# BoMingZhao/GaussianPrediction

Measured on AMD Instinct MI355X. Metric: rendered views/s (full train step) @1M Gaussians 1352x1014, higher is better.
Workload: dtype f32; 1 GPU; configs[2]: HyperNeRF-like 1M Gaussians, 1352x1014, stage-3 full train step (deform, raster, L1+SSIM loss, Adam: all HIP kernels); gaussians=1000000, width=1352, height=1014, keypoints=250, nearest_num=6, parallelism=view-parallel x1, ranks_seen_by_rccl=1, self_launched=False

## Files before the change

### gaussianprediction_amd/csrc/deform_kernels.h

```cpp
#pragma once
#include "gp_common.h"
#include "loss_adam_kernels.h"

struct MlpDev {
    long rows;
    int in_dim, in_pad, out_dim;
    int feature_dim, xyz_freq, time_freq;
    const float* w[5];
    const float* b[5];
    const float* feature;
    const float* xyz;
    const float* t;
    const float* pk;
};

struct MlpPackLayout {
    int q0;
    int tb0;
    long off_f[4], off_b[4], total;
};
static inline __host__ __device__ MlpPackLayout mlp_pack_layout(int in_dim) {
    MlpPackLayout L;
    L.q0 = (in_dim + 15) / 16;
    L.tb0 = 2 * ((in_dim + 31) / 32);
// ... 69 lines not shown
__global__ __launch_bounds__(1024) void gp_blend_bwd_reduce_kernel(const float* __restrict__ partial, int nblocks, int KA,
                                                                  int od, float* __restrict__ g_delta);
__global__ __launch_bounds__(256) void gp_act_fwd_kernel(long n, const float* __restrict__ scaling_raw,
                                                         const float* __restrict__ opacity_raw,
                                                         const float* __restrict__ delta_o, int stride, float beta,
                                                         float* __restrict__ scale, float* __restrict__ opacity);
__global__ __launch_bounds__(256) void gp_act_bwd_kernel(long n, const float* __restrict__ scaling_raw,
                                                         const float* __restrict__ opacity_raw,
                                                         const float* __restrict__ delta_o, int stride, float beta,
                                                         const float* __restrict__ g_scale,
                                                         const float* __restrict__ g_opacity,
                                                         float* __restrict__ g_scaling_raw, float* __restrict__ g_opacity_raw,
                                                         float* __restrict__ g_delta_o);

__global__ __launch_bounds__(512) void gp_mlp_bwd_weight5_kernel(MlpWeightJobs t, long rows);
__global__ __launch_bounds__(512) void gp_mlp_fwd_small_kernel(MlpDev p, float* __restrict__ out, float* __restrict__ saved_x,
                                                               float* __restrict__ saved_h);
__global__ __launch_bounds__(512) void gp_mlp_bwd_data_small_kernel(MlpDev p, const float* __restrict__ saved_h,
                                                                    const float* __restrict__ dL_dout, float* __restrict__ dz,
                                                                    float* __restrict__ dfeature, float* __restrict__ dxyz);

__global__ __launch_bounds__(256) void gp_mlp_fwd_split_small_kernel(MlpDev p, float* __restrict__ out, float* __restrict__ saved_x, float* hx,
                                                                     uint32_t* flags, uint32_t* err);
__global__ __launch_bounds__(256) void gp_mlp_fwd_split_small_agent_kernel(MlpDev p, float* __restrict__ out, float* __restrict__ saved_x,
                                                                           float* hx, uint32_t* flags, uint32_t* err);
__global__ __launch_bounds__(256) void gp_mlp_bwd_data_split_small_kernel(MlpDev p, const float* __restrict__ saved_h, const float* __restrict__ dL_dout,
                                                                          float* dz, float* __restrict__ dfeature, float* __restrict__ dxyz, float* gx,
                                                                          uint32_t* flags, uint32_t* err, int form);
struct AdamTable;
__global__ __launch_bounds__(512) void gp_mlp_bwd_data_small_adam_kernel(MlpDev p, const float* __restrict__ saved_h,
// ... 15 lines not shown
```

### gaussianprediction_amd/csrc/deform_kernels.hip

```cpp
#include "gp_common.h"
#include "deform_kernels.h"

typedef float f32x16 __attribute__((ext_vector_type(16)));

#define MLP_ROWS 32
#define MLP_THREADS 512
#define MLP_W 256

__device__ __forceinline__ int act_idx(int f, int j) { return f * MLP_ROWS + (j ^ (f & 31)); }
__device__ __forceinline__ int cd_row(int r, int half) { return (r & 3) + 8 * (r >> 2) + 4 * half; }

__device__ __forceinline__ void build_input(float* buf, const MlpDev& p, long row0, int tid) {
    const int fd = p.feature_dim, xf = p.xyz_freq, tf = p.time_freq;
    for (int e = tid; e < fd * MLP_ROWS; e += MLP_THREADS) {
        const int jj = e / fd, f = e - jj * fd;
        const long row = row0 + jj;
        buf[act_idx(f, jj)] = row < p.rows ? p.feature[row * fd + f] : 0.f;
    }
    for (int e = tid; e < 3 * xf * MLP_ROWS; e += MLP_THREADS) {
        const int jj = e % MLP_ROWS, cf = e / MLP_ROWS;
        const int c = cf / xf, fr = cf - c * xf;
        const long row = row0 + jj;
        float sv = 0.f, cv = 0.f;
        if (row < p.rows) {
// ... 407 lines not shown
                        for (int fr = 0; fr < p.xyz_freq; ++fr) {
                            const float sc = (float)(1u << fr);
                            float sv, cv;
                            sincosf(x * sc, &sv, &cv);
                            const int f = p.feature_dim + 2 * (c * p.xyz_freq + fr);
                            g += sc * (cv * buf[act_idx(f, jj)] - sv * buf[act_idx(f + 1, jj)]);
                        }
                        dxyz[row * 3 + c] = g;
                    }
                }
            }
        }
    }
}

__device__ __forceinline__ void mlp_bwd_weight_body(const float* __restrict__ dZ, int n_out, const float* __restrict__ H, int ldh,
                                                    int n_in, long rows, long rows_per_block, float* __restrict__ dW, int lddw,
                                                    float* __restrict__ db, int row_block, int n_row_blocks, int bz, int by) {
    __shared__ float s_red[8][16][64];
    __shared__ float s_b[8][32];
    const int tid = threadIdx.x, lane = tid & 63, wave = tid >> 6, half = lane >> 5, j = lane & 31;
    const int o = 32 * bz + j;
    const int i = 32 * by + j;
    const long b_begin = (long)row_block * rows_per_block;
    long b_end = b_begin + rows_per_block;
    if (b_end > rows) b_end = rows;
    long per_wave = ((b_end - b_begin + 7) / 8 + 1) & ~1L;
    const long r_begin = b_begin + wave * per_wave;
    long r_end = r_begin + per_wave;
    if (r_end > b_end) r_end = b_end;
    f32x16 acc;
#pragma unroll
    for (int r = 0; r < 16; ++r) acc[r] = 0.f;
// ... 5 lines not shown
        for (int u = 0; u < 4; ++u) {
            const long r = rb + 2 * u + half;
            a[u] = (r < r_end && o_ok) ? dZ[r * n_out + o] : 0.f;
            b[u] = (r < r_end && i_ok) ? H[r * (long)ldh + i] : 0.f;
            bsum += a[u];
        }
#pragma unroll
        for (int u = 0; u < 4; ++u) acc = __builtin_amdgcn_mfma_f32_32x32x2f32(a[u], b[u], acc, 0, 0, 0);
    }
#pragma unroll
    for (int r = 0; r < 16; ++r) s_red[wave][r][lane] = acc[r];
    bsum += __shfl_xor(bsum, 32);
    if (half == 0) s_b[wave][j] = bsum;
    __syncthreads();
    const bool single = n_row_blocks == 1;
    for (int e = tid; e < 16 * 64; e += MLP_THREADS) {
        const int r = e >> 6, l = e & 63;
        float v = 0.f;
#pragma unroll
        for (int w = 0; w < 8; ++w) v += s_red[w][r][l];
        const int oo = 32 * bz + cd_row(r, l >> 5), ii = 32 * by + (l & 31);
        if (oo < n_out && ii < n_in) {
            float* dst = &dW[(size_t)oo * lddw + ii];
            if (single) *dst += v; else atomicAdd(dst, v);
        }
    }
    if (db && by == 0 && tid < 32) {
        float v = 0.f;
#pragma unroll
        for (int w = 0; w < 8; ++w) v += s_b[w][tid];
        const int oo = 32 * bz + tid;
        if (oo < n_out) { if (single) db[oo] += v; else atomicAdd(&db[oo], v); }
    }
}

__global__ __launch_bounds__(MLP_THREADS) void gp_mlp_bwd_weight_kernel(const float* __restrict__ dZ, int n_out,
                                                                        const float* __restrict__ H, int ldh, int n_in,
                                                                        long rows, long rows_per_block,
                                                                        float* __restrict__ dW, int lddw,
                                                                        float* __restrict__ db) {
    mlp_bwd_weight_body(dZ, n_out, H, ldh, n_in, rows, rows_per_block, dW, lddw, db, blockIdx.x, gridDim.x, blockIdx.z, blockIdx.y);
}
__global__ __launch_bounds__(MLP_THREADS) void gp_mlp_bwd_weight5_kernel(MlpWeightJobs t, long rows) {
    const int l = blockIdx.x;
    if ((int)blockIdx.y * 32 >= t.n_in[l] || (int)blockIdx.z * 32 >= t.n_out[l]) return;
    mlp_bwd_weight_body(t.dZ[l], t.n_out[l], t.H[l], t.ldh[l], t.n_in[l], rows, rows, t.dW[l], t.n_in[l], t.db[l], 0, 1, blockIdx.z,
                        blockIdx.y);
}

__global__ __launch_bounds__(256) void gp_mlp_bwd_weight64_kernel(const float* __restrict__ dZ, int n_out, const float* __restrict__ H,
                                                                 int ldh, int n_in, long rows, long rows_per_block,
                                                                 unsigned n_row_blocks, float* __restrict__ dW, int lddw,
                                                                 float* __restrict__ db) {
    __shared__ float s_red[4][4][16][64];
    const int tid = threadIdx.x, lane = tid & 63, wave = tid >> 6, half = lane >> 5, j = lane & 31;
    const int n_ib = (n_in + 63) / 64;
    const int ntp = n_ib * ((n_out + 63) / 64);
    const unsigned flat = blockIdx.x, xcd = flat & 7u, seq = flat >> 3;
    const unsigned slab = (seq / ntp) * 8u + xcd, tp = seq % ntp;
    if (slab >= n_row_blocks) return;
    const int o0 = 64 * (tp / n_ib), i0 = 64 * (tp % n_ib);
    const long b_begin = (long)slab * rows_per_block;
// ... 436 lines not shown
            extern __shared__ float s_dyn[];
            double* s_tot = (double*)(((uintptr_t)s_dyn + 7) & ~(uintptr_t)7);
            loss_finalize_body(r.fin, (float*)(s_tot + 8), s_tot);
        } else {
            adam_chunk_body<256>(r.t, blockIdx.x - r.fin_blocks, threadIdx.x, r.b1, r.b2, r.eps, r.zero_grad, r.skip_flag);
        }
        return;
    }
    blend_bwd_body<NN, I16>(a, g_xyz_t, g_q_t, g_delta, g_raw_w, g_xyz, g_rot, partial, blockIdx.x - riders, gridDim.x - riders);
}
__global__ __launch_bounds__(256) void gp_blend_bwd6_ride_kernel(BlendRideDev r, BB_ARGS) { blend_bwd_ride_body<6, false>(r, a, g_xyz_t, g_q_t, g_delta, g_raw_w, g_xyz, g_rot, partial); }
__global__ __launch_bounds__(256) void gp_blend_bwd8_ride_kernel(BlendRideDev r, BB_ARGS) { blend_bwd_ride_body<8, false>(r, a, g_xyz_t, g_q_t, g_delta, g_raw_w, g_xyz, g_rot, partial); }
__global__ __launch_bounds__(256) void gp_blend_bwd6_i16_ride_kernel(BlendRideDev r, BB_ARGS) { blend_bwd_ride_body<6, true>(r, a, g_xyz_t, g_q_t, g_delta, g_raw_w, g_xyz, g_rot, partial); }
__global__ __launch_bounds__(256) void gp_blend_bwd8_i16_ride_kernel(BlendRideDev r, BB_ARGS) { blend_bwd_ride_body<8, true>(r, a, g_xyz_t, g_q_t, g_delta, g_raw_w, g_xyz, g_rot, partial); }

__global__ __launch_bounds__(1024) void gp_blend_bwd_reduce_kernel(const float* __restrict__ partial, int nblocks, int KA,
                                                                  int od, float* __restrict__ g_delta) {
    __shared__ float s_r[16][64];
    const int lane = threadIdx.x & 63, wave = threadIdx.x >> 6;
    const int e = blockIdx.x * 64 + lane;
    float v0 = 0.f, v1 = 0.f, v2 = 0.f, v3 = 0.f;
    if (e < KA) {
        int b = wave;
        for (; b + 240 < nblocks; b += 256) {
            float t[16];
#pragma unroll
            for (int u = 0; u < 16; ++u) t[u] = partial[(size_t)(b + 16 * u) * KA + e];
#pragma unroll
            for (int u = 0; u < 16; u += 4) { v0 += t[u]; v1 += t[u + 1]; v2 += t[u + 2]; v3 += t[u + 3]; }
        }
        for (; b + 48 < nblocks; b += 64) {
            v0 += partial[(size_t)b * KA + e]; v1 += partial[(size_t)(b + 16) * KA + e];
            v2 += partial[(size_t)(b + 32) * KA + e]; v3 += partial[(size_t)(b + 48) * KA + e];
        }
        for (; b < nblocks; b += 16) v0 += partial[(size_t)b * KA + e];
    }
    s_r[wave][lane] = (v0 + v1) + (v2 + v3);
    __syncthreads();
    if (wave == 0 && e < KA) {
        float t = 0.f;
#pragma unroll
        for (int w = 0; w < 16; ++w) t += s_r[w][lane];
        g_delta[(size_t)(e / 7) * od + (e % 7)] = t;
        if (e % 7 == 6) for (int c = 7; c < od; ++c) g_delta[(size_t)(e / 7) * od + c] = 0.f;
    }
}

__device__ __forceinline__ float sigmoidf(float x) { return 1.f / (1.f + expf(-x)); }

__global__ __launch_bounds__(256) void gp_act_fwd_kernel(long n, const float* __restrict__ scaling_raw,
                                                        const float* __restrict__ opacity_raw,
                                                        const float* __restrict__ delta_o, int stride, float beta,
                                                        float* __restrict__ scale, float* __restrict__ opacity) {
    const long i = (long)blockIdx.x * 256 + threadIdx.x;
    if (i >= n) return;
    const float s0 = scaling_raw[3 * i], s1 = scaling_raw[3 * i + 1], s2 = scaling_raw[3 * i + 2];
    const float op_raw = opacity_raw[i];
    const float dlt = delta_o ? delta_o[i * stride] : 0.f;
    scale[3 * i] = expf(s0);
    scale[3 * i + 1] = expf(s1);
// ... 32 lines not shown
```

### gaussianprediction_amd/csrc/gp_capi_deform.hip

```cpp
#include "gp_common.h"
#include "deform_kernels.h"
#include "loss_adam_kernels.h"
#include <stdlib.h>

static int make_mlp(const gp_mlp_params* p, const gp_mlp_input* x, MlpDev& m) {
    if (!p || !x) GP_FAIL("null mlp params/input");
    if (p->width != 256 || p->depth != 4) GP_FAIL("Deformable_Field: only d=4, w=256 is implemented (got d=%d w=%d)", p->depth, p->width);
    if (p->out_dim < 7 || p->out_dim > 8) GP_FAIL("out_dim must be 7 or 8 (got %d)", p->out_dim);
    if (x->feature_dim <= 0 || x->feature_dim % 4 || x->xyz_freq < 0 || x->xyz_freq > 16 || x->time_freq < 0 || x->time_freq > 16)
        GP_FAIL("bad input encoding dims");
    const int in_dim = x->feature_dim + 6 * x->xyz_freq + 2 * x->time_freq;
    if (in_dim != p->in_dim) GP_FAIL("in_dim %d != feature_dim + 6*xyz_freq + 2*time_freq = %d", p->in_dim, in_dim);
    if (in_dim % 4 || in_dim > 256) GP_FAIL("in_dim %d must be a multiple of 4 and <= 256", in_dim);
    if (x->rows < 0) GP_FAIL("negative rows");
    for (int l = 0; l < 5; ++l)
        if (!p->w[l] || !p->b[l]) GP_FAIL("null weight pointer (layer %d)", l);
    if (x->rows > 0 && (!x->feature || (x->xyz_freq > 0 && !x->xyz) || (x->time_freq > 0 && !x->t))) GP_FAIL("null input pointer");
    m.rows = x->rows; m.in_dim = in_dim; m.in_pad = (in_dim + 7) / 8 * 8; m.out_dim = p->out_dim;
    m.feature_dim = x->feature_dim; m.xyz_freq = x->xyz_freq; m.time_freq = x->time_freq;
    for (int l = 0; l < 5; ++l) { m.w[l] = p->w[l]; m.b[l] = p->b[l]; }
    m.feature = x->feature; m.xyz = x->xyz; m.t = x->t;
    m.pk = p->packed;
    if (m.pk && ((uintptr_t)m.pk & 15) != 0) GP_FAIL("gp_mlp_params.packed must be 16-byte aligned");
    if (p->scratch && ((uintptr_t)p->scratch & 15) != 0) GP_FAIL("gp_mlp_params.scratch must be 16-byte aligned");
// ... 96 lines not shown
            hipLaunchKernelGGL(gp_mlp_fwd_kernel, dim3(gp_blocks((size_t)m.rows, 32)), dim3(512), 0, (hipStream_t)stream_, m, out, sx, sh);
    GP_LAUNCH_CHECK(); }
    return 0;
}

bool gp_mlp_backward_splits(const gp_mlp_params* p, int64_t rows) {
    if (!p) return false;
    MlpDev m;
    memset(&m, 0, sizeof(m));
    m.rows = rows;
    int mode = 0;
    int* st = nullptr;
    return mlp_split_grid(m, p->scratch, mode, st) != 0 && (mode == 1 || mode == 3);
}

int gp_mlp_backward_impl(const gp_mlp_params* p, const gp_mlp_input* x, const float* acts, const float* dL_dout, gp_mlp_grads* g,
                         float* dL_dfeature, float* dL_dxyz, gp_alloc_fn alloc, void* alloc_ctx, gp_stream_t stream_, GpAdamRider* rider,
                         bool accumulate_dfeature) {
    hipStream_t s = (hipStream_t)stream_;
    MlpDev m;
    if (make_mlp(p, x, m)) return 1;
    if (m.rows == 0) return 0;
    if (!acts || !dL_dout || !g || !alloc) GP_FAIL("null argument");
    for (int l = 0; l < 5; ++l)
        if (!g->dw[l] || !g->db[l]) GP_FAIL("null weight-grad pointer (layer %d)", l);
    const float* sx = acts;
    const float* sh = acts + gp_align_up(acts_x_floats(m), 64);
    const size_t dz_bytes = gp_align_up((size_t)4 * m.rows * 256 * sizeof(float), 256);
    float* dz = (float*)alloc(alloc_ctx, GP_BUF_TEMP, dz_bytes);
    if (!dz) GP_FAIL("allocator returned NULL for TEMP (%zu B)", dz_bytes);
    int split_mode = 0;
    int* split_state = nullptr;
    const unsigned split = mlp_split_grid(m, p->scratch, split_mode, split_state);
    if (split && (split_mode == 1 || split_mode == 3)) {
        float* gx = (float*)((char*)p->scratch + GP_MLP_SCRATCH_FLAG_BYTES);
        uint32_t* flags = (uint32_t*)p->scratch;
        GpProfScope _p("mlp_bwd_data", s);
        hipLaunchKernelGGL(gp_mlp_bwd_data_split_small_kernel, dim3(split), dim3(256), 0, s, m, sh, dL_dout, dz, dL_dfeature, dL_dxyz, gx, flags,
                           flags + GP_MLP_SCRATCH_ERR_WORD, (split_mode == 3 ? 1 : 0) | (accumulate_dfeature ? 2 : 0));
        GP_LAUNCH_CHECK();
    } else if (m.rows <= GP_MLP_SMALL_ROWS && rider && rider->armed) {
        rider->armed = false;
        const unsigned n_mlp = gp_blocks((size_t)m.rows, 16);
        GpProfScope _p("adam", s);
        hipLaunchKernelGGL(gp_mlp_bwd_data_small_adam_kernel, dim3(n_mlp + rider->chunks), dim3(512), 0, s, m, sh, dL_dout, dz, dL_dfeature,
                           dL_dxyz, n_mlp, rider->t, rider->b1, rider->b2, rider->eps, rider->zero_grad, rider->skip_flag);
        GP_LAUNCH_CHECK();
    } else { GpProfScope _p("mlp_bwd_data", s);
        if (m.rows <= GP_MLP_SMALL_ROWS)
            hipLaunchKernelGGL(gp_mlp_bwd_data_small_kernel, dim3(gp_blocks((size_t)m.rows, 16)), dim3(512), 0, s, m, sh, dL_dout, dz,
                               dL_dfeature, dL_dxyz);
        else if (m.rows >= GP_MLP_LARGE_ROWS)
            hipLaunchKernelGGL(gp_mlp_bwd_data2_kernel, dim3(gp_blocks((size_t)m.rows, 64)), dim3(512), 0, s, m,
                               (const uint32_t*)(sh + (size_t)4 * m.rows * 256), dL_dout, dz,
                               dL_dfeature, dL_dxyz);
        else
            hipLaunchKernelGGL(gp_mlp_bwd_data_kernel, dim3(gp_blocks((size_t)m.rows, 32)), dim3(512), 0, s, m, sh, dL_dout, dz,
                       dL_dfeature, dL_dxyz);
    GP_LAUNCH_CHECK(); }
    long nrb_l = (m.rows + 4095) / 4096;
    if (nrb_l > 16) nrb_l = 16;
    if (nrb_l < 1) nrb_l = 1;
    long rpb = ((m.rows + nrb_l - 1) / nrb_l + 15) & ~15L;
    const unsigned nrb = (unsigned)((m.rows + rpb - 1) / rpb);
    GpProfScope _pw("mlp_bwd_weight", s);
    if (nrb == 1) {
        MlpWeightJobs jobs;
        for (int l = 0; l < 5; ++l) {
            jobs.dZ[l] = l < 4 ? dz + (size_t)l * m.rows * 256 : dL_dout;
            jobs.n_out[l] = l < 4 ? 256 : m.out_dim;
            jobs.H[l] = l == 0 ? sx : sh + (size_t)(l - 1) * m.rows * 256;
            jobs.ldh[l] = l == 0 ? m.in_pad : 256;
            jobs.n_in[l] = l == 0 ? m.in_dim : 256;
            jobs.dW[l] = g->dw[l]; jobs.db[l] = g->db[l];
        }
        hipLaunchKernelGGL(gp_mlp_bwd_weight5_kernel, dim3(5, 8, 8), dim3(512), 0, s, jobs, m.rows);
        GP_LAUNCH_CHECK();
        return 0;
    }
    if (m.rows >= 16384) {
        long nb = (m.rows + 4095) / 4096;
        if (nb < 64) nb = 64;
        const long brpb = ((m.rows + nb - 1) / nb + 7) & ~7L;
        const unsigned bnrb = (unsigned)((m.rows + brpb - 1) / brpb);
        for (int l = 0; l < 5; ++l) {
            const float* dZl = l < 4 ? dz + (size_t)l * m.rows * 256 : dL_dout;
            const int n_out = l < 4 ? 256 : m.out_dim;
            const float* H = l == 0 ? sx : sh + (size_t)(l - 1) * m.rows * 256;
            const int ldh = l == 0 ? m.in_pad : 256;
            const int n_in = l == 0 ? m.in_dim : 256;
            const unsigned ntp = (unsigned)((n_in + 63) / 64) * (unsigned)((n_out + 63) / 64);
// ... 7 lines not shown
        const float* dZl = l < 4 ? dz + (size_t)l * m.rows * 256 : dL_dout;
        const int n_out = l < 4 ? 256 : m.out_dim;
        const float* H = l == 0 ? sx : sh + (size_t)(l - 1) * m.rows * 256;
        const int ldh = l == 0 ? m.in_pad : 256;
        const int n_in = l == 0 ? m.in_dim : 256;
        {
        hipLaunchKernelGGL(gp_mlp_bwd_weight_kernel, dim3(nrb, (unsigned)((n_in + 31) / 32), (unsigned)((n_out + 31) / 32)),
                           dim3(512), 0, s, dZl, n_out, H, ldh, n_in, m.rows, rpb, g->dw[l], n_in, g->db[l]);
        GP_LAUNCH_CHECK(); }
    }
    return 0;
}
extern "C" int gp_mlp_backward(const gp_mlp_params* p, const gp_mlp_input* x, const float* acts, const float* dL_dout,
                               gp_mlp_grads* g, float* dL_dfeature, float* dL_dxyz, gp_alloc_fn alloc, void* alloc_ctx,
                               gp_stream_t stream_) {
    return gp_mlp_backward_impl(p, x, acts, dL_dout, g, dL_dfeature, dL_dxyz, alloc, alloc_ctx, stream_, nullptr, false);
}

static int make_blend(const gp_blend_args* a, BlendDev& b) {
    if (!a) GP_FAIL("null blend args");
    if (a->num_gaussians < 0) GP_FAIL("negative num_gaussians");
    if (a->out_dim < 7 || a->out_dim > 8) GP_FAIL("out_dim must be 7 or 8");
    if (a->nearest_num < 0 || a->nearest_num > 16) GP_FAIL("nearest_num %d unsupported (0..16)", a->nearest_num);
    if (a->nearest_num > 0 && (a->num_keypoints <= 0 || !a->raw_w || !a->knn_idx)) GP_FAIL("stage-2 blend needs keypoints, raw_w and knn_idx");
    if (a->nearest_num > 0 && a->num_keypoints * 7 * sizeof(float) > 60000) GP_FAIL("too many keypoints (%ld) for the LDS accumulator", (long)a->num_keypoints);
    if (a->num_gaussians > 0 && (!a->delta || !a->xyz || !a->rot)) GP_FAIL("null blend input");
    if (a->knn_idx16 && (a->num_keypoints > 65535 || ((uintptr_t)a->knn_idx16 & 3) != 0)) GP_FAIL("knn_idx16 needs K < 65536 and 4-byte alignment");
    b.N = a->num_gaussians; b.K = a->num_keypoints; b.nn = a->nearest_num; b.out_dim = a->out_dim;
    b.norm_rotation = a->norm_rotation; b.delta = a->delta; b.raw_w = a->raw_w; b.knn = a->knn_idx; b.xyz = a->xyz; b.rot = a->rot; b.knn16 = a->knn_idx16;
    return 0;
}
// ... 45 lines not shown
        }
        if (rider->fin_armed) { r.fin = rider->fin; r.fin_blocks = 1; }
        rider->adam.armed = rider->fin_armed = false;
        hipLaunchKernelGGL(b.nn == 6 ? (i16 ? gp_blend_bwd6_i16_ride_kernel : gp_blend_bwd6_ride_kernel)
                                     : (i16 ? gp_blend_bwd8_i16_ride_kernel : gp_blend_bwd8_ride_kernel),
                           dim3(r.fin_blocks + r.adam_chunks + blocks), dim3(256), lds, (hipStream_t)stream_, r, b, dL_dxyz_t, dL_dq_t, dL_ddelta,
                           dL_draw_w, dL_dxyz, dL_drot, partial);
    } else {
        hipLaunchKernelGGL(b.nn == 6 && al ? (i16 ? gp_blend_bwd6_i16_kernel : gp_blend_bwd6_kernel)
                           : b.nn == 8 && al ? (i16 ? gp_blend_bwd8_i16_kernel : gp_blend_bwd8_kernel) : gp_blend_bwd_kernel,
                           dim3(blocks), dim3(256), lds, (hipStream_t)stream_, b, dL_dxyz_t, dL_dq_t, dL_ddelta,
                           dL_draw_w, dL_dxyz, dL_drot, partial);
    }
    GP_LAUNCH_CHECK();
    if (b.nn > 0) {
        hipLaunchKernelGGL(gp_blend_bwd_reduce_kernel, dim3(gp_blocks((size_t)KA, 64)), dim3(1024), 0, (hipStream_t)stream_, partial,
                           (int)blocks, KA, b.out_dim, dL_ddelta);
        GP_LAUNCH_CHECK();
    } }
    return 0;
}
extern "C" int gp_blend_backward(const gp_blend_args* a, const float* dL_dxyz_t, const float* dL_dq_t, float* dL_ddelta,
                                 float* dL_draw_w, float* dL_dxyz, float* dL_drot, gp_alloc_fn alloc, void* alloc_ctx,
                                 gp_stream_t stream_) {
    return gp_blend_backward_impl(a, dL_dxyz_t, dL_dq_t, dL_ddelta, dL_draw_w, dL_dxyz, dL_drot, alloc, alloc_ctx, stream_, nullptr);
}

extern "C" int gp_activations_forward(int64_t n, const float* scaling_raw, const float* opacity_raw, const float* delta_o,
                                      int32_t stride, float beta, float* scale, float* opacity, gp_stream_t stream_) {
    if (n < 0) GP_FAIL("negative n");
    if (n == 0) return 0;
    if (!scaling_raw || !opacity_raw || !scale || !opacity) GP_FAIL("null argument");
// ... 19 lines not shown
```

### gaussianprediction_amd/csrc/gp_train_step.hip

```cpp
#include "gp_common.h"
#include "loss_adam_kernels.h"

__global__ __launch_bounds__(256) void gp_step_accumulate_kernel(float* __restrict__ dst, const float* __restrict__ src, int64_t n) {
    const int64_t i = (int64_t)blockIdx.x * 256 + threadIdx.x;
    if (i < n) dst[i] += src[i];
}

static int step_adam(const gp_step_update* u, uint32_t sel, gp_stream_t stream, GpAdamRider* ride = nullptr) {
    float *P[32], *G[32], *M[32], *V[32];
    int64_t NUM[32], ST[32];
    float LR[32];
    int n = 0;
    uint32_t keep = 0;
    for (int k = 0; k < u->adam_count && k < 32; ++k) {
        if (!((sel >> k) & 1u)) continue;
        P[n] = u->adam_params[k]; G[n] = u->adam_grads[k]; M[n] = u->adam_exp_avgs[k]; V[n] = u->adam_exp_avg_sqs[k];
        NUM[n] = u->adam_numels[k]; LR[n] = u->adam_lrs[k];
        ST[n] = u->adam_steps ? u->adam_steps[k] : u->step;
        if ((u->keep_grad_mask >> k) & 1u) keep |= 1u << n;
        ++n;
    }
    if (n == 0) return 0;
    if (ride) return gp_adam_rider_fill(ride, n, P, G, M, V, NUM, LR, ST, u->beta1, u->beta2, u->eps, 1, keep, u->skip_flag);
    return gp_adam_step_multi_steps(n, P, G, M, V, NUM, LR, ST, u->beta1, u->beta2, u->eps, 1, keep, u->skip_flag, stream);
// ... 56 lines not shown
    in.opacities = raw_act ? p->opacity : p->opacity_t;
    in.scales = raw_act ? p->scaling : p->scale; in.rotations = p->q_t;
    gp_raster_outputs out = p->out;
    gp_raster_saved saved;
    memset(&saved, 0, sizeof(saved));
    if (gp_raster_forward(&st, &in, &out, &saved, alloc, alloc_ctx, stream)) return 1;
    alloc(alloc_ctx, GP_BUF_TEMP_DONE, 0);
    if (u->hook) u->hook(u->hook_ctx, GP_STEP_AFTER_FORWARD);

    float* dimg = p->dL_dimage;
    if (!dimg) GP_FAIL("gp_train_step_run: null intermediate buffer");
    const int riders_off = gp_debug_get(15);
    GpLossPrologue pro;
    pro.armed = false;
    GpBlendRider blend_riders;
    blend_riders.fin_armed = blend_riders.adam.armed = false;
    if (gp_debug_get(11) == 0) {
        if (!(riders_off & 1)) {
            if (gp_raster_backward_prepare(&st, &in, &saved, alloc, alloc_ctx, &pro)) return 1;
            temp_open = pro.armed;
        }
        if (gp_loss_l1_ssim_fused_impl(out.color, v->gt_image, 3, H, W, p->lambda_dssim, nullptr, p->loss_sums, dimg, reg ? p->keypoint_features : nullptr,
                                       nfeat, p->reg_scale, reg ? p->g_keypoint_features : nullptr, stream, &pro)) return 1;
        if (!(riders_off & 2)) {
            if (gp_loss_finalize_fill(&blend_riders.fin, p->loss_sums, 3, H, W, p->lambda_dssim, reg ? p->keypoint_features : nullptr, nfeat,
                                      p->reg_scale, p->loss)) return 1;
            blend_riders.fin_armed = true;
        } else if (reg) { if (gp_loss_l1_ssim_finalize_reg(p->loss_sums, 3, H, W, p->lambda_dssim, p->keypoint_features, nfeat, p->reg_scale, p->loss, stream)) return 1; }
        else if (gp_loss_l1_ssim_finalize(p->loss_sums, 3, H, W, p->lambda_dssim, p->loss, stream)) return 1;
    } else {
        float* dmaps = p->dmaps;
// ... 17 lines not shown
    memset(&g, 0, sizeof(g));
    g.dL_dmeans3D = p->g_xyz_t; g.dL_dmeans2D = p->g_means2D; g.dL_dshs = p->g_features_dc; g.dL_dshs_rest = p->g_features_rest;
    g.dL_dopacities = raw_act ? p->g_opacity : p->g_opacity_t; g.dL_dscales = raw_act ? p->g_scaling : p->g_scale; g.dL_drotations = p->g_q_t; g.accumulate_shs = 0; g.adam_shs = u->adam_shs;
    if (gp_raster_backward_impl(&st, &in, &out, &saved, dimg, nullptr, &g, alloc, alloc_ctx, stream, pro.armed ? pro.acc : nullptr)) return 1;
    alloc(alloc_ctx, GP_BUF_TEMP_DONE, 0);
    temp_open = false;
    if (u->hook) u->hook(u->hook_ctx, GP_STEP_AFTER_RASTER_BACKWARD);
    if (!raw_act && gp_activations_backward(N, p->scaling, p->opacity, nullptr, 0, 1.f, p->g_scale, p->g_opacity_t, p->g_scaling, p->g_opacity, nullptr, stream))
        return 1;
    const uint32_t all = u->adam_count >= 32 ? 0xFFFFFFFFu : ((1u << u->adam_count) - 1u);
    uint32_t rode = 0;
    if (!(riders_off & 4) && raw_act && !u->hook)
        for (int k = 0; k < u->adam_count; ++k)
            if (u->adam_params[k] == p->scaling || u->adam_params[k] == p->opacity) rode |= 1u << k;
    if (rode && step_adam(u, rode, stream, &blend_riders.adam)) return 1;
    if (gp_blend_backward_impl(&ba, p->g_xyz_t, p->g_q_t, p->g_delta, nullptr, p->g_xyz, p->g_rotation, alloc, alloc_ctx, stream, &blend_riders)) return 1;
    alloc(alloc_ctx, GP_BUF_TEMP_DONE, 0);
    if (blend_riders.fin_armed && gp_loss_finalize_launch(blend_riders.fin, (hipStream_t)stream)) return 1;
    if (gp_adam_rider_launch(&blend_riders.adam, (hipStream_t)stream)) return 1;
    const uint32_t early = (u->hook || u->adam_count <= 0) ? 0u : (u->adam_early_mask & all & ~rode);
    GpAdamRider mlp_rider;
    mlp_rider.armed = false;
    if (early && step_adam(u, early, stream, &mlp_rider)) return 1;
    gp_mlp_grads mg = p->g_mlp;
    const bool add_in_place = reg && gp_mlp_backward_splits(&p->mlp, K);
    if (gp_mlp_backward_impl(&p->mlp, &mi, p->acts, p->g_delta, &mg, (reg && !add_in_place) ? p->g_feature_tmp : p->g_keypoint_features,
                             p->g_keypoints, alloc, alloc_ctx, stream, &mlp_rider, add_in_place)) return 1;
    if (gp_adam_rider_launch(&mlp_rider, (hipStream_t)stream)) return 1;
    if (reg && !add_in_place) {
        hipLaunchKernelGGL(gp_step_accumulate_kernel, dim3(gp_blocks((size_t)nfeat, 256)), dim3(256), 0, (hipStream_t)stream,
                           p->g_keypoint_features, (const float*)p->g_feature_tmp, nfeat);
        GP_LAUNCH_CHECK();
    }
    if (u->hook) u->hook(u->hook_ctx, GP_STEP_AFTER_BACKWARD);

    if (u->adam_count > 0 && step_adam(u, all & ~early & ~rode, stream)) return 1;
    return 0;
}
```

### gaussianprediction_amd/csrc/loss_adam_kernels.h

```cpp
#pragma once
#include "gp_common.h"

#define ADAM_MAX_TENSORS 32
#define ADAM_CHUNK 16384
struct AdamTable {
    float* p[ADAM_MAX_TENSORS];
    float* g[ADAM_MAX_TENSORS];
    float* m[ADAM_MAX_TENSORS];
    float* v[ADAM_MAX_TENSORS];
    unsigned long long n[ADAM_MAX_TENSORS];
    float step_size[ADAM_MAX_TENSORS];
    float bc2_sqrt[ADAM_MAX_TENSORS];
    unsigned keep_grad_mask;
    unsigned chunk_begin[ADAM_MAX_TENSORS + 1];
    int count;
};

template <int THREADS>
__device__ __forceinline__ void adam_chunk_body(const AdamTable& t, unsigned chunk, int tid, float b1, float b2, float eps, int zero_grad,
                                                const uint32_t* __restrict__ skip_flag) {
    const bool skip = skip_flag && *skip_flag != 0;
    int k = 0;
    while (k + 1 < t.count && chunk >= t.chunk_begin[k + 1]) ++k;
    const size_t base = (size_t)(chunk - t.chunk_begin[k]) * ADAM_CHUNK;
// ... 40 lines not shown
    }
}

struct GpAdamRider {
    AdamTable t;
    float b1, b2, eps;
    int zero_grad;
    const uint32_t* skip_flag;
    unsigned chunks;
    bool armed;
};
int gp_adam_rider_fill(GpAdamRider* r, int count, float* const* params, float* const* grads, float* const* exp_avgs,
                       float* const* exp_avg_sqs, const int64_t* numels, const float* lrs, const int64_t* steps, float beta1, float beta2,
                       float eps, int zero_grad, uint32_t keep_grad_mask, const uint32_t* skip_flag);
int gp_adam_rider_launch(GpAdamRider* r, hipStream_t s);
int gp_mlp_backward_impl(const gp_mlp_params* p, const gp_mlp_input* x, const float* acts, const float* dL_dout, gp_mlp_grads* g,
                         float* dL_dfeature, float* dL_dxyz, gp_alloc_fn alloc, void* alloc_ctx, gp_stream_t stream, GpAdamRider* rider,
                         bool accumulate_dfeature);
bool gp_mlp_backward_splits(const gp_mlp_params* p, int64_t rows);

__device__ __forceinline__ float block_sum_256(float v, float* s_red) {
#pragma unroll
    for (int d = 32; d >= 1; d >>= 1) v += __shfl_xor(v, d);
    const int lane = threadIdx.x & 63, wave = threadIdx.x >> 6;
    if (lane == 0) s_red[wave] = v;
    __syncthreads();
    return s_red[0] + s_red[1] + s_red[2] + s_red[3];
}
__device__ __forceinline__ void loss_slot_totals(const double* __restrict__ sums, int nslots, double* s_red , double& s0, double& s1) {
    const int tid = threadIdx.x;
    double a = 0.0, b = 0.0;
    const double2* s2 = reinterpret_cast<const double2*>(sums);
    for (int k0 = tid; k0 < nslots; k0 += 256 * 8) {
// ... 58 lines not shown
int gp_loss_finalize_launch(const LossFinalizeDev& f, hipStream_t s);

struct BlendRideDev {
    AdamTable t;
    float b1, b2, eps;
    int zero_grad;
    const uint32_t* skip_flag;
    unsigned adam_chunks;
    unsigned fin_blocks;
    LossFinalizeDev fin;
};
struct GpBlendRider {
    GpAdamRider adam;
    LossFinalizeDev fin;
    bool fin_armed;
};
int gp_blend_backward_impl(const gp_blend_args* a, const float* dL_dxyz_t, const float* dL_dq_t, float* dL_ddelta, float* dL_draw_w,
                           float* dL_dxyz, float* dL_drot, gp_alloc_fn alloc, void* alloc_ctx, gp_stream_t stream, GpBlendRider* riders);

struct GpLossPrologue {
    const int2* ranges;
    const int32_t* tile_work;
    int T;
    uint32_t* order;
    float* acc;
    size_t acc_floats;
    bool armed;
};
int gp_raster_backward_prepare(const gp_raster_settings* st, const gp_raster_inputs* in, const gp_raster_saved* saved, gp_alloc_fn alloc,
                               void* alloc_ctx, GpLossPrologue* pro);
// ... 7 lines not shown
```

### gaussianprediction_amd/csrc/loss_adam_kernels.hip

```cpp
#include "gp_common.h"
#include "loss_adam_kernels.h"
#include "raster_kernels.h"

#define GP_LOSS_REG_MAX 65536
#define LT 32
#define LH 5
#define LE (LT + 2 * LH)
#define LP (LE + 1)
#define LHP (LT + 1)

struct Win11 { float w[11]; };

__global__ __launch_bounds__(256) void gp_l1_ssim_fwd_kernel(const float* __restrict__ img, const float* __restrict__ gt,
                                                            int H, int W, Win11 win, double* __restrict__ sums,
                                                            float* __restrict__ dmap) {
    __shared__ float s_a[LE][LP], s_b[LE][LP];
    __shared__ float s_h[4][LE][LHP];
    __shared__ float s_red[4];
    const int tid = threadIdx.x;
    const int tx0 = blockIdx.x * LT, ty0 = blockIdx.y * LT, ch = blockIdx.z;
    const size_t HW = (size_t)H * W;
    const float* a_img = img + ch * HW;
    const float* b_img = gt + ch * HW;
    {
// ... 551 lines not shown
    if (count < 0 || count > ADAM_MAX_TENSORS) GP_FAIL("adam: at most %d tensors per call (got %d)", ADAM_MAX_TENSORS, count);
    if (count == 0) return 0;
    if (!params || !grads || !exp_avgs || !exp_avg_sqs || !numels || !lrs || !steps) GP_FAIL("null argument");
    t.count = 0;
    t.keep_grad_mask = 0;
    unsigned chunks = 0;
    for (int k = 0; k < count; ++k) {
        if (numels[k] <= 0) continue;
        if (steps[k] < 1) GP_FAIL("adam: bad step %lld (tensor %d)", (long long)steps[k], k);
        if ((((uintptr_t)params[k] | (uintptr_t)grads[k] | (uintptr_t)exp_avgs[k] | (uintptr_t)exp_avg_sqs[k]) & 15) != 0)
            GP_FAIL("adam: pointers must be 16-byte aligned (tensor %d)", k);
        const int j = t.count++;
        if ((keep_grad_mask >> k) & 1u) t.keep_grad_mask |= 1u << j;
        t.p[j] = params[k]; t.g[j] = grads[k]; t.m[j] = exp_avgs[k]; t.v[j] = exp_avg_sqs[k];
        t.n[j] = (unsigned long long)numels[k];
        t.step_size[j] = lrs[k] / (1.f - powf(beta1, (float)steps[k]));
        t.bc2_sqrt[j] = sqrtf(1.f - powf(beta2, (float)steps[k]));
        t.chunk_begin[j] = chunks;
        chunks += (unsigned)((numels[k] + ADAM_CHUNK - 1) / ADAM_CHUNK);
    }
    t.chunk_begin[t.count] = chunks;
    n_chunks = (long)chunks;
    return 0;
}

int gp_adam_rider_fill(GpAdamRider* r, int count, float* const* params, float* const* grads, float* const* exp_avgs,
                       float* const* exp_avg_sqs, const int64_t* numels, const float* lrs, const int64_t* steps, float beta1, float beta2,
                       float eps, int zero_grad, uint32_t keep_grad_mask, const uint32_t* skip_flag) {
    r->armed = false;
    long chunks = 0;
    if (adam_build_table(r->t, chunks, count, params, grads, exp_avgs, exp_avg_sqs, numels, lrs, steps, beta1, beta2, keep_grad_mask)) return 1;
    r->b1 = beta1; r->b2 = beta2; r->eps = eps; r->zero_grad = zero_grad; r->skip_flag = skip_flag; r->chunks = (unsigned)chunks;
// ... 56 lines not shown
```

Measured before the change: 867.8 views/s.

## Ride Adam updates on blend reduce and MLP weight-gradient kernels

Adds 'ride' variants of the blend backward reduce kernel and the 5-layer MLP weight-gradient kernel. Extra blocks in these launches run Adam chunks for xyz, rotation and keypoint tensors. The MLP weight kernel can also apply Adam directly to the MLP weights and biases while it writes their gradients, which removes separate Adam launches and a re-read of the gradients. In exchange the host-side tensor matching and masking logic becomes more complex, and the grids become larger and mixed-purpose, which could skew load balance.

```diff
diff --git a/gaussianprediction_amd/csrc/deform_kernels.h b/gaussianprediction_amd/csrc/deform_kernels.h
--- a/gaussianprediction_amd/csrc/deform_kernels.h
+++ b/gaussianprediction_amd/csrc/deform_kernels.h
@@ -107,6 +107,16 @@
                                                          float* __restrict__ g_delta_o);
 
 __global__ __launch_bounds__(512) void gp_mlp_bwd_weight5_kernel(MlpWeightJobs t, long rows);
+struct TailRideDev {
+    AdamTable t;
+    float b1, b2, eps;
+    int zero_grad;
+    const uint32_t* skip_flag;
+    unsigned own_blocks;
+};
+__global__ __launch_bounds__(1024) void gp_blend_bwd_reduce_ride_kernel(TailRideDev r, const float* __restrict__ partial, int nblocks, int KA,
+                                                                       int od, float* __restrict__ g_delta);
+__global__ __launch_bounds__(512) void gp_mlp_bwd_weight5_ride_kernel(TailRideDev r, MlpWeightAdam a, MlpWeightJobs t, long rows);
 __global__ __launch_bounds__(512) void gp_mlp_fwd_small_kernel(MlpDev p, float* __restrict__ out, float* __restrict__ saved_x,
                                                                float* __restrict__ saved_h);
 __global__ __launch_bounds__(512) void gp_mlp_bwd_data_small_kernel(MlpDev p, const float* __restrict__ saved_h,
diff --git a/gaussianprediction_amd/csrc/deform_kernels.hip b/gaussianprediction_amd/csrc/deform_kernels.hip
--- a/gaussianprediction_amd/csrc/deform_kernels.hip
+++ b/gaussianprediction_amd/csrc/deform_kernels.hip
@@ -445,9 +445,17 @@
     }
 }
 
+__device__ __forceinline__ void mlp_weight_adam_elem(const MlpWeightAdam& a, int layer, int j, size_t idx, float* dst, float v, bool skip) {
+    const float g = *dst + v;
+    if (!skip) gp_adam_update(a.p[layer][j][idx], g, a.m[layer][j][idx], a.v[layer][j][idx], a.b1, a.b2, a.eps, a.step_size[layer][j],
+                              a.bc2_sqrt[layer][j]);
+    *dst = ((a.keep_mask >> (2 * layer + j)) & 1u) ? g : 0.f;
+}
+template <bool ADAM = false>
 __device__ __forceinline__ void mlp_bwd_weight_body(const float* __restrict__ dZ, int n_out, const float* __restrict__ H, int ldh,
                                                     int n_in, long rows, long rows_per_block, float* __restrict__ dW, int lddw,
-                                                    float* __restrict__ db, int row_block, int n_row_blocks, int bz, int by) {
+                                                    float* __restrict__ db, int row_block, int n_row_blocks, int bz, int by,
+                                                    const MlpWeightAdam* adam = nullptr, int layer = 0) {
     __shared__ float s_red[8][16][64];
     __shared__ float s_b[8][32];
     const int tid = threadIdx.x, lane = tid & 63, wave = tid >> 6, half = lane >> 5, j = lane & 31;
@@ -483,6 +491,8 @@
     if (half == 0) s_b[wave][j] = bsum;
     __syncthreads();
     const bool single = n_row_blocks == 1;
+    const bool upd = ADAM && adam->on;
+    const bool skip = upd && adam->skip_flag && *adam->skip_flag != 0;
     for (int e = tid; e < 16 * 64; e += MLP_THREADS) {
         const int r = e >> 6, l = e & 63;
         float v = 0.f;
@@ -491,7 +501,8 @@
         const int oo = 32 * bz + cd_row(r, l >> 5), ii = 32 * by + (l & 31);
         if (oo < n_out && ii < n_in) {
             float* dst = &dW[(size_t)oo * lddw + ii];
-            if (single) *dst += v; else atomicAdd(dst, v);
+            if (upd) mlp_weight_adam_elem(*adam, layer, 0, (size_t)oo * lddw + ii, dst, v, skip);
+            else if (single) *dst += v; else atomicAdd(dst, v);
         }
     }
     if (db && by == 0 && tid < 32) {
@@ -499,7 +510,10 @@
 #pragma unroll
         for (int w = 0; w < 8; ++w) v += s_b[w][tid];
         const int oo = 32 * bz + tid;
-        if (oo < n_out) { if (single) db[oo] += v; else atomicAdd(&db[oo], v); }
+        if (oo < n_out) {
+            if (upd) mlp_weight_adam_elem(*adam, layer, 1, (size_t)oo, &db[oo], v, skip);
+            else if (single) db[oo] += v; else atomicAdd(&db[oo], v);
+        }
     }
 }
 
@@ -515,6 +529,15 @@
     if ((int)blockIdx.y * 32 >= t.n_in[l] || (int)blockIdx.z * 32 >= t.n_out[l]) return;
     mlp_bwd_weight_body(t.dZ[l], t.n_out[l], t.H[l], t.ldh[l], t.n_in[l], rows, rows, t.dW[l], t.n_in[l], t.db[l], 0, 1, blockIdx.z,
                         blockIdx.y);
+}
+__global__ __launch_bounds__(MLP_THREADS) void gp_mlp_bwd_weight5_ride_kernel(TailRideDev r, MlpWeightAdam a, MlpWeightJobs t, long rows) {
+    if (blockIdx.x >= r.own_blocks) {
+        adam_chunk_body<MLP_THREADS>(r.t, blockIdx.x - r.own_blocks, threadIdx.x, r.b1, r.b2, r.eps, r.zero_grad, r.skip_flag);
+        return;
+    }
+    const int l = blockIdx.x % 5, by = (blockIdx.x / 5) & 7, bz = blockIdx.x / 40;
+    if (by * 32 >= t.n_in[l] || bz * 32 >= t.n_out[l]) return;
+    mlp_bwd_weight_body<true>(t.dZ[l], t.n_out[l], t.H[l], t.ldh[l], t.n_in[l], rows, rows, t.dW[l], t.n_in[l], t.db[l], 0, 1, bz, by, &a, l);
 }
 
 __global__ __launch_bounds__(256) void gp_mlp_bwd_weight64_kernel(const float* __restrict__ dZ, int n_out, const float* __restrict__ H,
@@ -981,8 +1004,8 @@
 __global__ __launch_bounds__(256) void gp_blend_bwd6_i16_ride_kernel(BlendRideDev r, BB_ARGS) { blend_bwd_ride_body<6, true>(r, a, g_xyz_t, g_q_t, g_delta, g_raw_w, g_xyz, g_rot, partial); }
 __global__ __launch_bounds__(256) void gp_blend_bwd8_i16_ride_kernel(BlendRideDev r, BB_ARGS) { blend_bwd_ride_body<8, true>(r, a, g_xyz_t, g_q_t, g_delta, g_raw_w, g_xyz, g_rot, partial); }
 
-__global__ __launch_bounds__(1024) void gp_blend_bwd_reduce_kernel(const float* __restrict__ partial, int nblocks, int KA,
-                                                                  int od, float* __restrict__ g_delta) {
+__device__ __forceinline__ void blend_bwd_reduce_body(const float* __restrict__ partial, int nblocks, int KA, int od,
+                                                      float* __restrict__ g_delta) {
     __shared__ float s_r[16][64];
     const int lane = threadIdx.x & 63, wave = threadIdx.x >> 6;
     const int e = blockIdx.x * 64 + lane;
@@ -1011,6 +1034,18 @@
         g_delta[(size_t)(e / 7) * od + (e % 7)] = t;
         if (e % 7 == 6) for (int c = 7; c < od; ++c) g_delta[(size_t)(e / 7) * od + c] = 0.f;
     }
+}
+__global__ __launch_bounds__(1024) void gp_blend_bwd_reduce_kernel(const float* __restrict__ partial, int nblocks, int KA,
+                                                                  int od, float* __restrict__ g_delta) {
+    blend_bwd_reduce_body(partial, nblocks, KA, od, g_delta);
+}
+__global__ __launch_bounds__(1024) void gp_blend_bwd_reduce_ride_kernel(TailRideDev r, const float* __restrict__ partial, int nblocks, int KA,
+                                                                       int od, float* __restrict__ g_delta) {
+    if (blockIdx.x >= r.own_blocks) {
+        adam_chunk_body<1024>(r.t, blockIdx.x - r.own_blocks, threadIdx.x, r.b1, r.b2, r.eps, r.zero_grad, r.skip_flag);
+        return;
+    }
+    blend_bwd_reduce_body(partial, nblocks, KA, od, g_delta);
 }
 
 __device__ __forceinline__ float sigmoidf(float x) { return 1.f / (1.f + expf(-x)); }
diff --git a/gaussianprediction_amd/csrc/gp_capi_deform.hip b/gaussianprediction_amd/csrc/gp_capi_deform.hip
--- a/gaussianprediction_amd/csrc/gp_capi_deform.hip
+++ b/gaussianprediction_amd/csrc/gp_capi_deform.hip
@@ -134,9 +134,17 @@
     return mlp_split_grid(m, p->scratch, mode, st) != 0 && (mode == 1 || mode == 3);
 }
 
+static void tail_ride_take(TailRideDev& r, GpAdamRider* rider, unsigned own_blocks) {
+    memset(&r, 0, sizeof(r));
+    r.own_blocks = own_blocks;
+    if (!rider || !rider->armed) return;
+    r.t = rider->t; r.b1 = rider->b1; r.b2 = rider->b2; r.eps = rider->eps; r.zero_grad = rider->zero_grad; r.skip_flag = rider->skip_flag;
+    rider->armed = false;
+}
+
 int gp_mlp_backward_impl(const gp_mlp_params* p, const gp_mlp_input* x, const float* acts, const float* dL_dout, gp_mlp_grads* g,
                          float* dL_dfeature, float* dL_dxyz, gp_alloc_fn alloc, void* alloc_ctx, gp_stream_t stream_, GpAdamRider* rider,
-                         bool accumulate_dfeature) {
+                         bool accumulate_dfeature, bool weight_host, GpMlpAdamRider* wadam) {
     hipStream_t s = (hipStream_t)stream_;
     MlpDev m;
     if (make_mlp(p, x, m)) return 1;
@@ -152,7 +160,9 @@
     int split_mode = 0;
     int* split_state = nullptr;
     const unsigned split = mlp_split_grid(m, p->scratch, split_mode, split_state);
+    bool split_data = false;
     if (split && (split_mode == 1 || split_mode == 3)) {
+        split_data = true;
         float* gx = (float*)((char*)p->scratch + GP_MLP_SCRATCH_FLAG_BYTES);
         uint32_t* flags = (uint32_t*)p->scratch;
         GpProfScope _p("mlp_bwd_data", s);
@@ -183,7 +193,9 @@
     if (nrb_l < 1) nrb_l = 1;
     long rpb = ((m.rows + nrb_l - 1) / nrb_l + 15) & ~15L;
     const unsigned nrb = (unsigned)((m.rows + rpb - 1) / rpb);
-    GpProfScope _pw("mlp_bwd_weight", s);
+    const bool chunks = nrb == 1 && weight_host && split_data && rider && rider->armed;
+    const bool inside = nrb == 1 && weight_host && split_data && wadam && wadam->armed;
+    GpProfScope _pw(chunks || inside ? "adam" : "mlp_bwd_weight", s);
     if (nrb == 1) {
         MlpWeightJobs jobs;
         for (int l = 0; l < 5; ++l) {
@@ -194,7 +206,17 @@
             jobs.n_in[l] = l == 0 ? m.in_dim : 256;
             jobs.dW[l] = g->dw[l]; jobs.db[l] = g->db[l];
         }
-        hipLaunchKernelGGL(gp_mlp_bwd_weight5_kernel, dim3(5, 8, 8), dim3(512), 0, s, jobs, m.rows);
+        if (chunks || inside) {
+            TailRideDev r;
+            const unsigned n_chunks = chunks ? rider->chunks : 0u;
+            tail_ride_take(r, chunks ? rider : nullptr, 5 * 8 * 8);
+            MlpWeightAdam a;
+            memset(&a, 0, sizeof(a));
+            if (inside) { a = wadam->d; a.on = 1; wadam->armed = false; }
+            hipLaunchKernelGGL(gp_mlp_bwd_weight5_ride_kernel, dim3(5 * 8 * 8 + n_chunks), dim3(512), 0, s, r, a, jobs, m.rows);
+        } else {
+            hipLaunchKernelGGL(gp_mlp_bwd_weight5_kernel, dim3(5, 8, 8), dim3(512), 0, s, jobs, m.rows);
+        }
         GP_LAUNCH_CHECK();
         return 0;
     }
@@ -232,7 +254,7 @@
 extern "C" int gp_mlp_backward(const gp_mlp_params* p, const gp_mlp_input* x, const float* acts, const float* dL_dout,
                                gp_mlp_grads* g, float* dL_dfeature, float* dL_dxyz, gp_alloc_fn alloc, void* alloc_ctx,
                                gp_stream_t stream_) {
-    return gp_mlp_backward_impl(p, x, acts, dL_dout, g, dL_dfeature, dL_dxyz, alloc, alloc_ctx, stream_, nullptr, false);
+    return gp_mlp_backward_impl(p, x, acts, dL_dout, g, dL_dfeature, dL_dxyz, alloc, alloc_ctx, stream_, nullptr, false, false, nullptr);
 }
 
 static int make_blend(const gp_blend_args* a, BlendDev& b) {
@@ -308,8 +330,17 @@
     }
     GP_LAUNCH_CHECK();
     if (b.nn > 0) {
-        hipLaunchKernelGGL(gp_blend_bwd_reduce_kernel, dim3(gp_blocks((size_t)KA, 64)), dim3(1024), 0, (hipStream_t)stream_, partial,
-                           (int)blocks, KA, b.out_dim, dL_ddelta);
+        const unsigned rblocks = gp_blocks((size_t)KA, 64);
+        if (rider && rider->tail.armed) {
+            TailRideDev r;
+            const unsigned n_chunks = rider->tail.chunks;
+            tail_ride_take(r, &rider->tail, rblocks);
+            hipLaunchKernelGGL(gp_blend_bwd_reduce_ride_kernel, dim3(rblocks + n_chunks), dim3(1024), 0, (hipStream_t)stream_, r, partial,
+                               (int)blocks, KA, b.out_dim, dL_ddelta);
+        } else {
+            hipLaunchKernelGGL(gp_blend_bwd_reduce_kernel, dim3(rblocks), dim3(1024), 0, (hipStream_t)stream_, partial, (int)blocks, KA,
+                               b.out_dim, dL_ddelta);
+        }
         GP_LAUNCH_CHECK();
     } }
     return 0;
diff --git a/gaussianprediction_amd/csrc/gp_train_step.hip b/gaussianprediction_amd/csrc/gp_train_step.hip
--- a/gaussianprediction_amd/csrc/gp_train_step.hip
+++ b/gaussianprediction_amd/csrc/gp_train_step.hip
@@ -94,7 +94,7 @@
     GpLossPrologue pro;
     pro.armed = false;
     GpBlendRider blend_riders;
-    blend_riders.fin_armed = blend_riders.adam.armed = false;
+    blend_riders.fin_armed = blend_riders.adam.armed = blend_riders.tail.armed = false;
     if (gp_debug_get(11) == 0) {
         if (!(riders_off & 1)) {
             if (gp_raster_backward_prepare(&st, &in, &saved, alloc, alloc_ctx, &pro)) return 1;
@@ -142,19 +142,66 @@
         for (int k = 0; k < u->adam_count; ++k)
             if (u->adam_params[k] == p->scaling || u->adam_params[k] == p->opacity) rode |= 1u << k;
     if (rode && step_adam(u, rode, stream, &blend_riders.adam)) return 1;
+    const bool splits = gp_mlp_backward_splits(&p->mlp, K);
+    const bool add_in_place = reg && splits;
+    const bool tail_ok = !u->hook && raw_act && u->adam_count > 0 && splits;
+    uint32_t tail_reduce = 0, tail_weight = 0, tail_inside = 0;
+    GpMlpAdamRider mlp_adam;
+    mlp_adam.armed = false;
+    if (tail_ok && !(riders_off & 8))
+        for (int k = 0; k < u->adam_count; ++k) {
+            if (u->adam_numels[k] <= 0 || ((rode >> k) & 1u)) continue;
+            if (u->adam_params[k] == p->xyz && u->adam_grads[k] == p->g_xyz) tail_reduce |= 1u << k;
+            if (u->adam_params[k] == p->rotation && u->adam_grads[k] == p->g_rotation) tail_weight |= 1u << k;
+        }
+    if (tail_ok && !(riders_off & 16)) {
+        if (!reg || add_in_place)
+            for (int k = 0; k < u->adam_count; ++k) {
+                if (u->adam_numels[k] <= 0) continue;
+                if ((u->adam_params[k] == p->keypoints && u->adam_grads[k] == p->g_keypoints) ||
+                    (u->adam_params[k] == p->keypoint_features && u->adam_grads[k] == p->g_keypoint_features)) tail_weight |= 1u << k;
+            }
+        MlpWeightAdam& d = mlp_adam.d;
+        memset(&d, 0, sizeof(d));
+        bool all_found = true;
+        for (int l = 0; l < 5 && all_found; ++l)
+            for (int j = 0; j < 2 && all_found; ++j) {
+                const float* param = j == 0 ? p->mlp.w[l] : p->mlp.b[l];
+                const float* grad = j == 0 ? p->g_mlp.dw[l] : p->g_mlp.db[l];
+                const int64_t n_out = l < 4 ? p->mlp.width : p->mlp.out_dim, n_in = l == 0 ? p->mlp.in_dim : p->mlp.width;
+                int k = 0;
+                while (k < u->adam_count && !(u->adam_params[k] == param && u->adam_grads[k] == grad &&
+                                              u->adam_numels[k] == (j == 0 ? n_out * n_in : n_out) && !((tail_inside >> k) & 1u))) ++k;
+                if (k == u->adam_count) { all_found = false; break; }
+                const int64_t st = u->adam_steps ? u->adam_steps[k] : u->step;
+                if (st < 1) { all_found = false; break; }
+                tail_inside |= 1u << k;
+                d.p[l][j] = u->adam_params[k]; d.m[l][j] = u->adam_exp_avgs[k]; d.v[l][j] = u->adam_exp_avg_sqs[k];
+                gp_adam_bias(u->adam_lrs[k], u->beta1, u->beta2, st, d.step_size[l][j], d.bc2_sqrt[l][j]);
+                if ((u->keep_grad_mask >> k) & 1u) d.keep_mask |= 1u << (2 * l + j);
+            }
+        if (all_found && p->mlp.width == 256) {
+            d.b1 = u->beta1; d.b2 = u->beta2; d.eps = u->eps; d.skip_flag = u->skip_flag;
+            mlp_adam.armed = true;
+        } else {
+            tail_inside = 0;
+        }
+    }
+    if (tail_reduce && step_adam(u, tail_reduce, stream, &blend_riders.tail)) return 1;
     if (gp_blend_backward_impl(&ba, p->g_xyz_t, p->g_q_t, p->g_delta, nullptr, p->g_xyz, p->g_rotation, alloc, alloc_ctx, stream, &blend_riders)) return 1;
     alloc(alloc_ctx, GP_BUF_TEMP_DONE, 0);
     if (blend_riders.fin_armed && gp_loss_finalize_launch(blend_riders.fin, (hipStream_t)stream)) return 1;
     if (gp_adam_rider_launch(&blend_riders.adam, (hipStream_t)stream)) return 1;
-    const uint32_t early = (u->hook || u->adam_count <= 0) ? 0u : (u->adam_early_mask & all & ~rode);
+    if (gp_adam_rider_launch(&blend_riders.tail, (hipStream_t)stream)) return 1;
+    const uint32_t early = ((u->hook || u->adam_count <= 0) ? 0u : (u->adam_early_mask & all & ~rode & ~tail_reduce)) | tail_weight;
     GpAdamRider mlp_rider;
     mlp_rider.armed = false;
     if (early && step_adam(u, early, stream, &mlp_rider)) return 1;
     gp_mlp_grads mg = p->g_mlp;
-    const bool add_in_place = reg && gp_mlp_backward_splits(&p->mlp, K);
     if (gp_mlp_backward_impl(&p->mlp, &mi, p->acts, p->g_delta, &mg, (reg && !add_in_place) ? p->g_feature_tmp : p->g_keypoint_features,
-                             p->g_keypoints, alloc, alloc_ctx, stream, &mlp_rider, add_in_place)) return 1;
+                             p->g_keypoints, alloc, alloc_ctx, stream, &mlp_rider, add_in_place, tail_weight != 0 || mlp_adam.armed, &mlp_adam)) return 1;
     if (gp_adam_rider_launch(&mlp_rider, (hipStream_t)stream)) return 1;
+    if (mlp_adam.armed) tail_inside = 0;
     if (reg && !add_in_place) {
         hipLaunchKernelGGL(gp_step_accumulate_kernel, dim3(gp_blocks((size_t)nfeat, 256)), dim3(256), 0, (hipStream_t)stream,
                            p->g_keypoint_features, (const float*)p->g_feature_tmp, nfeat);
@@ -162,6 +209,6 @@
     }
     if (u->hook) u->hook(u->hook_ctx, GP_STEP_AFTER_BACKWARD);
 
-    if (u->adam_count > 0 && step_adam(u, all & ~early & ~rode, stream)) return 1;
+    if (u->adam_count > 0 && step_adam(u, all & ~early & ~rode & ~tail_reduce & ~tail_inside, stream)) return 1;
     return 0;
 }
diff --git a/gaussianprediction_amd/csrc/loss_adam_kernels.h b/gaussianprediction_amd/csrc/loss_adam_kernels.h
--- a/gaussianprediction_amd/csrc/loss_adam_kernels.h
+++ b/gaussianprediction_amd/csrc/loss_adam_kernels.h
@@ -78,9 +78,25 @@
                        float* const* exp_avg_sqs, const int64_t* numels, const float* lrs, const int64_t* steps, float beta1, float beta2,
                        float eps, int zero_grad, uint32_t keep_grad_mask, const uint32_t* skip_flag);
 int gp_adam_rider_launch(GpAdamRider* r, hipStream_t s);
+struct MlpWeightAdam {
+    float* p[5][2]; float* m[5][2]; float* v[5][2];
+    float step_size[5][2], bc2_sqrt[5][2];
+    unsigned keep_mask;
+    float b1, b2, eps;
+    const uint32_t* skip_flag;
+    int on;
+};
+struct GpMlpAdamRider {
+    MlpWeightAdam d;
+    bool armed;
+};
+inline void gp_adam_bias(float lr, float beta1, float beta2, int64_t step, float& step_size, float& bc2_sqrt) {
+    step_size = lr / (1.f - powf(beta1, (float)step));
+    bc2_sqrt = sqrtf(1.f - powf(beta2, (float)step));
+}
 int gp_mlp_backward_impl(const gp_mlp_params* p, const gp_mlp_input* x, const float* acts, const float* dL_dout, gp_mlp_grads* g,
                          float* dL_dfeature, float* dL_dxyz, gp_alloc_fn alloc, void* alloc_ctx, gp_stream_t stream, GpAdamRider* rider,
-                         bool accumulate_dfeature);
+                         bool accumulate_dfeature, bool weight_host = false, GpMlpAdamRider* wadam = nullptr);
 bool gp_mlp_backward_splits(const gp_mlp_params* p, int64_t rows);
 
 __device__ __forceinline__ float block_sum_256(float v, float* s_red) {
@@ -169,6 +185,7 @@
     GpAdamRider adam;
     LossFinalizeDev fin;
     bool fin_armed;
+    GpAdamRider tail;
 };
 int gp_blend_backward_impl(const gp_blend_args* a, const float* dL_dxyz_t, const float* dL_dq_t, float* dL_ddelta, float* dL_draw_w,
                            float* dL_dxyz, float* dL_drot, gp_alloc_fn alloc, void* alloc_ctx, gp_stream_t stream, GpBlendRider* riders);
diff --git a/gaussianprediction_amd/csrc/loss_adam_kernels.hip b/gaussianprediction_amd/csrc/loss_adam_kernels.hip
--- a/gaussianprediction_amd/csrc/loss_adam_kernels.hip
+++ b/gaussianprediction_amd/csrc/loss_adam_kernels.hip
@@ -589,8 +589,7 @@
         if ((keep_grad_mask >> k) & 1u) t.keep_grad_mask |= 1u << j;
         t.p[j] = params[k]; t.g[j] = grads[k]; t.m[j] = exp_avgs[k]; t.v[j] = exp_avg_sqs[k];
         t.n[j] = (unsigned long long)numels[k];
-        t.step_size[j] = lrs[k] / (1.f - powf(beta1, (float)steps[k]));
-        t.bc2_sqrt[j] = sqrtf(1.f - powf(beta2, (float)steps[k]));
+        gp_adam_bias(lrs[k], beta1, beta2, steps[k], t.step_size[j], t.bc2_sqrt[j]);
         t.chunk_begin[j] = chunks;
         chunks += (unsigned)((numels[k] + ADAM_CHUNK - 1) / ADAM_CHUNK);
     }
```

New measurement: 872.7 views/s, median of 6. No clear change (+0.6%).
